# mihikamd/DP-GSAT

Hardware: AMD Instinct MI355X
Metric: million edges/s (attn+sample+aggregate fwd+bwd) (higher is better)
Workload: dtype f32

## Files before the change

### dp_gsat_amd/_lib.py

```python
from __future__ import annotations

import ctypes
import os
from ctypes import c_char_p, c_double, c_float, c_int, c_int32, c_int64, c_size_t, c_uint64, c_void_p

import torch

_HERE = os.path.dirname(os.path.abspath(__file__))
LIB_PATH = os.path.join(_HERE, "libgsat_hip.so")

P, I64, I32, F32, F64, SZ, INT, U64 = c_void_p, c_int64, c_int32, c_float, c_double, c_size_t, c_int, c_uint64

SIGNATURES = {
    "gsat_abi_version": (INT, []),
    "gsat_seed_next": (INT, [P, P, P]),
    "gsat_last_error": (c_char_p, []),
    "gsat_csr_workspace_bytes": (SZ, [I64, I64]),
    "gsat_rev_workspace_bytes": (SZ, [I64]),
    "gsat_build_csr": (INT, [P, P, I64, I64, P, P, P, P, P, SZ, P]),
    "gsat_reverse_edge_perm": (INT, [P, I64, I64, P, P, P, SZ, P]),
    "gsat_reverse_edge_perm_csr": (INT, [P, P, P, P, P, P, P, P, I64, I64, P, P, P]),
    "gsat_segment_ptr": (INT, [P, I64, I64, P, P, P]),
    "gsat_gather_i64": (INT, [P, I64, P, I64, P, P]),
    "gsat_row_chunks_workspace_bytes": (SZ, [I64]),
    "gsat_row_chunks": (INT, [P, I64, P, P, SZ, P]),
    "gsat_long_row_partial_floats": (SZ, [I64, I64]),
    "gsat_aggr_sum_fwd": (INT, [P, P, P, P, P, P, P, I64, I64, I64, F32, P, P, P, P]),
    "gsat_aggr_sum_bwd": (INT, [P, P, P, P, P, P, P, I64, I64, I64, F32, P, P, P, P, P, P]),
    "gsat_pna_fwd": (INT, [P, P, P, P, P, P, I64, I64, P, INT, P, INT, F32, F32, P, P]),
    "gsat_pna_bwd": (INT, [P, P, P, P, P, P, P, I64, I64, P, INT, P, INT, F32, F32, P, P, P, P, P]),
    "gsat_pna_long_row_floats": (SZ, [I64, I64, INT]),
    "gsat_pna_fwd_long": (INT, [P, P, P, P, P, P, I64, I64, I64, P, INT, P, INT, F32, F32, P, P, P, P]),
    "gsat_pna_bwd_long": (INT, [P, P, P, P, P, P, P, I64, I64, I64, P, INT, P, INT, F32, F32, P, P, P, P, P, P, P]),
    "gsat_pna_tile_plan": (INT, [I64, I64, P, P, P]),
    "gsat_pna_build_tiles": (INT, [P, P, P, P, P, I64, INT, INT, INT, P, P, P, P]),
    "gsat_pna_bwd_tiled": (INT, [P, P, P, P, P, P, P, I64, INT, INT, INT, P, P, I64, I64, I64, P, INT, P, INT, P, P, P, P, P, P, P]),
    "gsat_pna_fwd_compact": (INT, [P, P, P, P, P, I64, I64, P, INT, P, P, P]),
    "gsat_pna_post_fwd": (INT, [P, P, P, I64, I64, INT, P, I64, P, I64, P, P]),
    "gsat_pna_post_dw_workspace_floats": (SZ, [I64, I64, INT, I64]),
    "gsat_pna_post_dw": (INT, [P, P, P, I64, I64, INT, P, I64, P, P, SZ, P]),
    "gsat_pna_fwd_node_att": (INT, [P, P, P, P, I64, I64, P, INT, P, INT, F32, F32, P, P]),
    "gsat_pna_bwd_tiled_node_att": (INT, [P, P, P, P, P, P, I64, INT, INT, INT, P, P, I64, I64, I64, P, INT, P, INT, P, P, P, P, P, P, P, INT, P]),
    "gsat_csr_pair_workspace_bytes": (SZ, [I64, I64]),
    "gsat_build_csr_pair": (INT, [P, I64, I64] + [P] * 12 + [P, SZ, P]),
    "gsat_segment_ptr32": (INT, [P, I64, I64, P, P, P, P]),
    "gsat_bn_workspace_floats": (SZ, [I64, I64]),
    "gsat_bn_fwd": (INT, [P, P, P, P, P, I64, I64, INT, F32, F32, INT, P, P, P, P, P]),
    "gsat_bn_bwd": (INT, [P, P, P, P, P, P, I64, I64, INT, INT, P, P, P, P, P]),
    "gsat_bn_act_fwd": (INT, [P, P, P, P, P, I64, I64, INT, F32, F32, INT, P, F32, U64, P, P, P, P, P, P]),
    "gsat_bn_act_bwd": (INT, [P, P, P, P, P, P, I64, I64, INT, INT, F32, U64, P, P, P, P, P, P, P]),
    "gsat_bn_act_fwd_valid": (INT, [P, P, P, P, P, I64, I64, INT, F32, F32, INT, P, F32, U64, P, P, P, P, P, P, P]),
    "gsat_bn_act_bwd_valid": (INT, [P, P, P, P, P, P, I64, I64, INT, INT, F32, U64, P, P, P, P, P, P, P, P]),
    "gsat_bn_local_sum": (INT, [P, P, I64, I64, P, P, P]),
    "gsat_bn_apply_fwd": (INT, [P, P, P, P, P, I64, I64, INT, P, F32, U64, P, P, P]),
    "gsat_bn_local_bwd_sums": (INT, [P, P, P, P, P, P, I64, I64, INT, F32, U64, P, P, P, P, P]),
    "gsat_bn_apply_bwd": (INT, [P, P, P, P, P, P, P, P, I64, P, I64, I64, INT, F32, U64, P, P, P, P]),
    "gsat_relu_dropout_fwd": (INT, [P, I64, I64, F32, U64, P, P, P]),
    "gsat_relu_dropout_bwd": (INT, [P, P, I64, I64, F32, P, P]),
    "gsat_colsum_workspace_floats": (SZ, [I64]),
    "gsat_colsum": (INT, [P, I64, I64, P, P, P]),
    "gsat_embsum_fwd": (INT, [P, P, INT, P, I64, I64, P, P]),
    "gsat_onehot_rows": (INT, [P, P, INT, I64, I64, P, P]),
    "gsat_gemm_workspace_floats": (SZ, [INT, I64, I64, I64]),
    "gsat_gemm_plan": (INT, [INT, INT, INT, I64, I64, I64, INT, INT, I64, P]),
    "gsat_gemm_f32": (INT, [INT, INT, I64, I64, I64, P, I64, P, I64, P, I64, P, INT, P, SZ, P]),
    "gsat_gemm_bf16x3": (INT, [INT, INT, I64, I64, I64, P, I64, P, I64, P, I64, P, INT, P, SZ, P]),
    "gsat_attn_fwd_workspace_bytes": (SZ, [P]),
    "gsat_attn_fwd_kind": (I32, [P]),
    "gsat_attn_bwd_workspace_bytes": (SZ, [P]),
    "gsat_attn_fwd": (INT, [P, P]),
    "gsat_attn_bwd": (INT, [P, P, P]),
    "gsat_instance_norm_fwd": (INT, [P, P, P, P, I64, I64, I64, P, P, P]),
    "gsat_instance_norm_bwd": (INT, [P, P, P, P, P, P, I64, I64, I64, P, P, P]),
    "gsat_philox_keep_mask": (INT, [U64, I32, I64, I64, F32, P, P]),
    "gsat_philox_noise": (INT, [U64, I64, P, P]),
    "gsat_sample_fwd": (INT, [P, P, INT, F32, F32, I64, P, P]),
    "gsat_sample_bwd": (INT, [P, P, F32, I64, P, P]),
    "gsat_gumbel_sigmoid_philox": (INT, [P, I64, F32, F32, U64, P, P, P]),
    "gsat_philox_gumbel_noise": (INT, [U64, I64, P, P]),
    "gsat_lift_fwd": (INT, [P, P, P, I64, P, P]),
    "gsat_lift_bwd": (INT, [P, P, P, P, P, P, P, P, I64, P, P]),
    "gsat_symmetrise": (INT, [P, P, P, I64, P, P]),
    "gsat_info_loss_fwd": (INT, [P, P, F32, I64, P, P, P]),
    "gsat_info_loss_bwd": (INT, [P, P, F32, P, I64, P, P]),
    "gsat_info_loss_valid_fwd": (INT, [P, P, F32, P, I64, P, P, P, P]),
    "gsat_info_loss_valid_bwd": (INT, [P, P, F32, P, P, I64, P, P, P]),
    "gsat_f1_sparsity_fwd": (INT, [P, P, I64, P, P, P, P, P]),
    "gsat_f1_sparsity_bwd": (INT, [P, P, P, P, I64, P, P, P]),
    "gsat_f1_sparsity_block_entries": (I64, []),
    "gsat_f1_sparsity_max_blocks": (I64, []),
    "gsat_criterion_fwd": (INT, [P, P, I64, I64, INT, P, P, P, P, P]),
    "gsat_criterion_bwd": (INT, [P, P, P, P, I64, I64, INT, P, P, P]),
    "gsat_criterion_block_items": (I64, [I64, INT]),
    "gsat_criterion_max_blocks": (I64, []),
    "gsat_ragged_scan": (INT, [P, I64, P, P, I64, P, P, P, P, P, P]),
    "gsat_collate_padded_ragged": (INT, [P, I64, P, P, P, P, I64, P, P, I64, I64, P, P, P, P, P, P]),
    "gsat_collate_padded": (INT, [P, I64, P, P, P, I64, P, P, I64, I64, P, P, P, P, P, P]),
    "gsat_collate": (INT, [P, I64, P, P, P, I64, P, P, I64, I64, P, P, P, P, P]),
    "gsat_line_graph_pair_counts": (INT, [P, I64, P, P]),
    "gsat_line_graph": (INT, [P, P, P, I64, I64, P, P]),
    "gsat_narrow_i64": (INT, [P, I64, P, P]),
    "gsat_und_edges_workspace_bytes": (SZ, [I64]),
    "gsat_und_edges": (INT, [P, I64, I64, P, P, P, P, P, P, P, P, SZ, P]),
    "gsat_und_line_graph_counts": (INT, [P, P, P, P, I64, P, P]),
    "gsat_und_line_graph": (INT, [P, P, P, P, P, I64, I64, P, P]),
    "gsat_segment_pool_fwd": (INT, [P, P, I64, I64, INT, P, P]),
    "gsat_segment_pool_bwd": (INT, [P, P, I64, I64, INT, P, P]),
    "gsat_rank_edges_lds_cap": (I64, []),
    "gsat_rank_edges_workspace_bytes": (SZ, [I64]),
    "gsat_rank_edges": (INT, [P, P, P, P, I64, I64, I64, I64, INT, P, P, P, P, P, SZ, P]),
    "gsat_auroc_workspace_bytes": (SZ, [I64]),
    "gsat_auroc": (INT, [P, P, I64, P, P, SZ, P]),
    "gsat_delta_kl_workspace_bytes": (SZ, [I64]),
    "gsat_delta_kl": (INT, [P, P, I64, F64, P, P, SZ, P]),
    "gsat_auroc_tasks_workspace_bytes": (SZ, [I64, I64]),
    "gsat_auroc_tasks": (INT, [P, P, I64, I64, P, P, SZ, P]),
    "gsat_att_histogram": (INT, [P, P, I64, I64, F64, F64, P, P, P]),
    "gsat_subgraph_block_items": (I64, []),
    "gsat_subgraph_workspace_bytes": (SZ, [I64, I64]),
# ... 79 lines not shown
```

### dp_gsat_amd/csrc/attn.hip

```cpp
#include "common.h"
#include "attn_fused.h"
#include <cstdlib>

namespace gsat {

constexpr float IN_EPS = 1e-5f;
constexpr int SB = 256;
#ifndef GSAT_SB_LANES
#define GSAT_SB_LANES 16
#endif
constexpr int SB_LANES = GSAT_SB_LANES;
constexpr int SB_SLOTS = SB / SB_LANES;
constexpr int SB_RC = 2;

struct GemmWs { float* ptr; size_t floats; };
static int gemm_rm(hipStream_t stream, bool ta, bool tb, int64_t M, int64_t N, int64_t K, const float* A, int64_t lda, const float* B,
                   int64_t ldb, float beta, float* C, int64_t ldc, GemmWs ws = {nullptr, 0}, bool split_ok = false, SlabJob* defer = nullptr) {
    const char* env = getenv("GSAT_ATTN_BWD_SPLIT");
    const bool bwd_split = !(env && atoi(env) == 0);
    return gemm_f32(stream, ta, tb, M, N, K, A, lda, B, ldb, C, ldc, nullptr, beta != 0.f, ws.ptr, ws.floats, split_ok && bwd_split, defer);
}

template <bool EDGE>
struct PreAct {
    const float* P; const float* Q; const float* bias; const int32_t* src; const int32_t* dst; int C;
    __device__ __forceinline__ float4 load(int row, int c) const {
        float4 b = bias ? ld4(bias + c) : f4zero();
        float4 v;
        if (EDGE) {
            float4 p = ld4(P + (size_t)src[row] * C + c);
            float4 q = ld4(Q + (size_t)dst[row] * C + c);
            v = make_float4(p.x + q.x, p.y + q.y, p.z + q.z, p.w + q.w);
        } else {
            v = ld4(P + (size_t)row * C + c);
        }
        return make_float4(v.x + b.x, v.y + b.y, v.z + b.z, v.w + b.w);
    }
};

__device__ __forceinline__ float4 keep4(const float* mask, SeedRef sref, int layer, int row, int c, int C, float p, bool training) {
    if (!training || p <= 0.f) return make_float4(1.f, 1.f, 1.f, 1.f);
    if (mask) return ld4(mask + (size_t)row * C + c);
    return philox_keep4(sref.get(), layer, row, c, p);
}

__device__ __forceinline__ float4 slot_reduce(float4 v, float4 (*sm)[SB_LANES], int slot, int lane) {
    __syncthreads();
    sm[slot][lane] = v;
    __syncthreads();
    float4 r = f4zero();
    if (slot == 0) {
#pragma unroll
        for (int s = 0; s < SB_SLOTS; ++s) {
            float4 t = sm[s][lane];
            r.x += t.x; r.y += t.y; r.z += t.z; r.w += t.w;
        }
    }
    return r;
}

__device__ __forceinline__ void seg_slice(const int32_t* __restrict__ seg_ptr, int g, int* beg, int* end, float* inv_n) {
    const int b = seg_ptr[g], e = seg_ptr[g + 1];
    *inv_n = 1.f / (float)max(e - b, 1);
    const int Z = gridDim.z, z = blockIdx.z;
    if (Z > 1) {
        const int per = (e - b + Z - 1) / Z;
        *beg = min(e, b + z * per);
        *end = min(e, *beg + per);
    } else {
        *beg = b; *end = e;
    }
}
// ... 542 lines not shown
        const int m = (int)(i / C4), c = (int)(i % C4) * 4;
        st4(keep + (size_t)m * C + c, keep4(nullptr, SeedRef{seed, nullptr}, layer, m, c, C, p, true));
    }
}

static inline int ew_blocks(int64_t work_items) {
    int64_t nb = ceil_div(work_items, 256);
    if (nb > 256 * 32) nb = 256 * 32;
    return (int)std::max<int64_t>(nb, 1);
}

static int colsum(hipStream_t stream, const float* x, int64_t R, int C, float* out, float* scratch ) {
    if (C <= 0) return GSAT_OK;
    const int ctiles = (int)ceil_div(C, 4 * SB_LANES);
    if (R <= 0) { GSAT_CHECK_HIP(gsat::zero_async(out, sizeof(float) * C, stream)); return GSAT_OK; }
    int64_t RB = std::min<int64_t>(256, ceil_div(R, 64));
    if (RB <= 1) {
        k_colsum<<<dim3(ctiles, 1), SB, 0, stream>>>(x, R, C, R, out);
    } else {
        int64_t rpb = ceil_div(R, RB);
        RB = ceil_div(R, rpb);
        k_colsum<<<dim3(ctiles, (unsigned)RB), SB, 0, stream>>>(x, R, C, rpb, scratch);
        k_colsum<<<dim3(ctiles, 1), SB, 0, stream>>>(scratch, RB, C, RB, out);
    }
    GSAT_LAUNCH_CHECK();
    return GSAT_OK;
}

static inline int seg_slices(int64_t rows, int64_t G) {
    const int64_t avg = rows / std::max<int64_t>(G, 1);
    return (int)std::max<int64_t>(1, std::min<int64_t>(64, ceil_div(avg, 4096)));
}

template <bool EDGE>
static int launch_seg_stats(hipStream_t stream, PreAct<EDGE> pre, const int32_t* seg_ptr, const int32_t* order, int64_t G, int Z,
                            float* mean, float* rstd, float* part) {
    if (G <= 0) return GSAT_OK;
    const int C = pre.C;
    const dim3 grid((unsigned)G, (unsigned)ceil_div(C, 4 * SB_LANES), (unsigned)Z);
    if (Z == 1) {
        k_seg_stats<EDGE, false><<<grid, SB, 0, stream>>>(pre, seg_ptr, order, mean, rstd);
    } else {
        GSAT_REQUIRE(part, GSAT_ERR_WORKSPACE, "segmented statistics need a workspace for sliced segments");
        const unsigned cb = (unsigned)ceil_div(G * C, 256);
        k_seg_partial<EDGE><<<grid, SB, 0, stream>>>(pre, seg_ptr, order, nullptr, part);
        k_zcombine<<<cb, 256, 0, stream>>>(part, seg_ptr, (int)G, Z, C, 1, mean);
        k_seg_partial<EDGE><<<grid, SB, 0, stream>>>(pre, seg_ptr, order, mean, part);
        k_zcombine<<<cb, 256, 0, stream>>>(part, seg_ptr, (int)G, Z, C, 2, rstd);
    }
    GSAT_LAUNCH_CHECK();
    return GSAT_OK;
}

static size_t attn_gemm_ws_w2(const gsat_attn_args* a) { return align_up(gemm_workspace_floats(a->C2, a->C1, a->M, true), 64); }
static size_t attn_gemm_ws_w1(const gsat_attn_args* a) { return align_up(gemm_workspace_floats(a->C1, a->H, a->N, true), 64); }
static size_t attn_gemm_ws_floats(const gsat_attn_args* a) { return attn_gemm_ws_w2(a) + (a->edge_mode ? 2 : 1) * attn_gemm_ws_w1(a); }

static int check_args(const gsat_attn_args* a, const char* who) {
    GSAT_REQUIRE(a, GSAT_ERR_ARG, "%s: null args", who);
    GSAT_REQUIRE(a->M >= 0 && a->N >= 0 && a->G >= 0 && a->M < (1ll << 31) && a->N < (1ll << 31), GSAT_ERR_ARG, "%s: bad extents", who);
    GSAT_REQUIRE(a->H > 0 && a->C1 > 0 && a->C2 > 0 && a->H % 4 == 0 && a->C1 % 4 == 0 && a->C2 % 4 == 0, GSAT_ERR_UNSUPPORTED,
                 "%s: H, C1, C2 must be positive multiples of 4 (got %d, %d, %d)", who, a->H, a->C1, a->C2);
    GSAT_REQUIRE(a->p_drop >= 0.f && a->p_drop < 1.f, GSAT_ERR_ARG, "%s: dropout p must be in [0,1)", who);
    if (a->M == 0) return GSAT_OK;
    GSAT_REQUIRE(a->emb && a->W1 && a->b1 && a->W2 && a->b2 && a->W3 && a->b3 && a->seg_ptr && a->row_seg, GSAT_ERR_ARG, "%s: null input", who);
    GSAT_REQUIRE(a->P && a->h2 && a->stats && a->logits, GSAT_ERR_ARG, "%s: null output/saved buffer", who);
    if (a->edge_mode) GSAT_REQUIRE(a->src && a->dst && a->Q, GSAT_ERR_ARG, "%s: edge mode needs src, dst, Q", who);
    else GSAT_REQUIRE(a->M == a->N, GSAT_ERR_ARG, "%s: node mode needs M == N", who);
    return GSAT_OK;
}

}

using namespace gsat;

extern "C" {

size_t gsat_colsum_workspace_floats(int64_t C) { return (size_t)256 * (size_t)(C > 0 ? C : 0); }

int gsat_colsum(const float* x, int64_t R, int64_t C, float* out, float* workspace, void* stream) {
    GSAT_REQUIRE(R >= 0 && C >= 0 && C < (1ll << 31), GSAT_ERR_ARG, "gsat_colsum: bad extents");
    if (C == 0) return GSAT_OK;
    GSAT_REQUIRE(out && (x || R == 0) && workspace, GSAT_ERR_ARG, "gsat_colsum: null pointer");
    return colsum((hipStream_t)stream, x, R, (int)C, out, workspace);
}


int gsat_attn_fwd(const gsat_attn_args* a, void* stream_) {
    hipStream_t stream = (hipStream_t)stream_;
    int rc = check_args(a, "gsat_attn_fwd");
    if (rc) return rc;
    if (a->M == 0) return GSAT_OK;
    {
        FusedGeom fg;
        if (attn_fused_eligible(a, &fg)) return attn_fused_fwd(stream, a, fg);
    }
    GSAT_REQUIRE(a->a1, GSAT_ERR_ARG, "gsat_attn_fwd: the staged pipeline needs the a1 buffer");
    const int64_t M = a->M, N = a->N, G = a->G;
    const int H = a->H, C1 = a->C1, C2 = a->C2;
    float* mean1 = a->stats;
    float* rstd1 = mean1 + (size_t)G * C1;
    float* mean2 = rstd1 + (size_t)G * C1;
    float* rstd2 = mean2 + (size_t)G * C2;
    if (a->edge_mode) {
        if ((rc = gemm_rm(stream, false, true, N, C1, H, a->emb, H, a->W1, 2 * H, 0.f, a->P, C1))) return rc;
        if ((rc = gemm_rm(stream, false, true, N, C1, H, a->emb, H, a->W1 + H, 2 * H, 0.f, a->Q, C1))) return rc;
    } else {
        if ((rc = gemm_rm(stream, false, true, N, C1, H, a->emb, H, a->W1, H, 0.f, a->P, C1))) return rc;
// ... 281 lines not shown
```

### dp_gsat_amd/csrc/common.h

```cpp
#pragma once
#include <cstring>
#include <cstdint>
#include <cstdio>
#include <cstdarg>
#include <hip/hip_runtime.h>

#include "../../include/gsat_hip.h"

namespace gsat {

void set_error(const char* fmt, ...);
const char* get_error();

#define GSAT_CHECK_HIP(expr)                                                                  \
    do {                                                                                      \
        hipError_t _e = (expr);                                                               \
        if (_e != hipSuccess) {                                                               \
            gsat::set_error("%s:%d: %s -> %s", __FILE__, __LINE__, #expr, hipGetErrorString(_e)); \
            return GSAT_ERR_HIP;                                                              \
        }                                                                                     \
    } while (0)

#define GSAT_REQUIRE(cond, code, ...)                                                         \
    do {                                                                                      \
        if (!(cond)) {                                                                        \
            gsat::set_error(__VA_ARGS__);                                                     \
            return (code);                                                                    \
        }                                                                                     \
    } while (0)

#define GSAT_LAUNCH_CHECK() GSAT_CHECK_HIP(hipGetLastError())

static inline int64_t ceil_div(int64_t a, int64_t b) { return (a + b - 1) / b; }

hipError_t zero_async(void* p, size_t bytes, hipStream_t stream);
static inline size_t align_up(size_t a, size_t b) { return (a + b - 1) / b * b; }

struct Arena {
    char* base;
    size_t cap, off;
    Arena(void* p, size_t bytes) : base(static_cast<char*>(p)), cap(bytes), off(0) {}
    template <class T> T* take(size_t n) {
        size_t b = align_up(n * sizeof(T), 256);
        if (base == nullptr || off + b > cap) { off += b; return nullptr; }
        T* r = reinterpret_cast<T*>(base + off);
        off += b;
        return r;
    }
    bool ok() const { return base != nullptr && off <= cap; }
};

struct SlabJob { const float* ws; int nslab; size_t slab; int M, N; int64_t ldc; int accumulate; float* out; };
int gemm_f32(hipStream_t stream, bool a_t, bool b_t, int64_t M, int64_t N, int64_t K, const float* A, int64_t lda, const float* B,
             int64_t ldb, float* C, int64_t ldc, const float* bias, bool accumulate, float* ws, size_t ws_floats, bool allow_split = false,
             SlabJob* defer = nullptr);
int slab_reduce_jobs(hipStream_t stream, const SlabJob* jobs, int n);
size_t gemm_workspace_floats(int64_t M, int64_t N, int64_t K, bool reduce_rows);

int aggr_sum_fwd_impl(hipStream_t stream, const float* x, const float* self_rows, const float* att, const float* edge_emb,
                      const int32_t* rowptr, const int32_t* col, const int32_t* eid, int64_t N, int64_t E, int64_t H, float self_coef,
                      float* out, const int32_t* chunk_ptr, float* partial);

#ifdef __HIPCC__
constexpr int WAVE = 64;

template <int CTRL> __device__ __forceinline__ float dpp_add(float v) {
    const int t = __builtin_amdgcn_update_dpp(0, __builtin_bit_cast(int, v), CTRL, 0xF, 0xF, true);
    return v + __builtin_bit_cast(float, t);
}

template <int WIDTH> __device__ __forceinline__ float group_sum(float v) {
    if constexpr ((WIDTH & (WIDTH - 1)) == 0) {
        if constexpr (WIDTH >= 2) v = dpp_add<0xB1>(v);
        if constexpr (WIDTH >= 4) v = dpp_add<0x4E>(v);
        if constexpr (WIDTH >= 8) v = dpp_add<0x141>(v);
        if constexpr (WIDTH >= 16) v = dpp_add<0x140>(v);
        if constexpr (WIDTH >= 32) v += __builtin_bit_cast(float, __builtin_amdgcn_ds_swizzle(__builtin_bit_cast(int, v), 0x401F));
        if constexpr (WIDTH >= 64) v += __shfl_xor(v, 32, 64);
    } else {
        const int l = (int)(threadIdx.x & 63) % WIDTH;
#pragma unroll
        for (int o = 16; o > 0; o >>= 1) {
            const float t = __shfl_down(v, o, 64);
            if (l + o < WIDTH) v += t;
        }
    }
    return v;
}

template <int LPR, int BLOCK> struct LaneGroups {
    static constexpr int GPW = 64 / LPR, GPB = (BLOCK / 64) * GPW;
    int grp, lane;
    __device__ __forceinline__ LaneGroups() {
        const int wl = threadIdx.x & 63, sub = wl / LPR;
        lane = wl % LPR;
        grp = sub < GPW ? (int)(threadIdx.x >> 6) * GPW + sub : -1;
    }
};

__device__ __forceinline__ float4 ld4(const float* p) { return *reinterpret_cast<const float4*>(p); }
__device__ __forceinline__ void st4(float* p, float4 v) { *reinterpret_cast<float4*>(p) = v; }
__device__ __forceinline__ void st4_nt(float* p, float4 v) {
    typedef float v4f __attribute__((ext_vector_type(4)));
    v4f t = {v.x, v.y, v.z, v.w};
    __builtin_nontemporal_store(t, reinterpret_cast<v4f*>(p));
}
__device__ __forceinline__ float4 ld4_off(const float* base, uint32_t byte_off) {
    return *reinterpret_cast<const float4*>(reinterpret_cast<const char*>(base) + byte_off);
}
__device__ __forceinline__ void st4_off(float* base, uint32_t byte_off, float4 v) {
// ... 55 lines not shown
```

### dp_gsat_amd/csrc/gemm.hip

```cpp
#include "common.h"
#include "pna_math.h"
#include <cstdlib>

namespace gsat {

typedef float f32x16 __attribute__((ext_vector_type(16)));

constexpr int GK = 32, GT = 256;
constexpr int LD_KC = 129;
constexpr int LD_KM = 132;

struct StageKC { float4 v[4]; };
template <int ROWS>
__device__ __forceinline__ void load_kcontig(StageKC& s, const float* __restrict__ X, int64_t ld, int r0, int R, int k0, int K, int t) {
    const int kq = (t & 7) * 4;
#pragma unroll
    for (int p = 0; p < ROWS / 32; ++p) {
        const int r = r0 + (t >> 3) + 32 * p;
        s.v[p] = (r < R && k0 + kq < K) ? ld4(X + (size_t)r * ld + k0 + kq) : f4zero();
    }
}
template <int ROWS>
__device__ __forceinline__ void store_kcontig(const StageKC& s, float* __restrict__ L, int t) {
    const int kq = (t & 7) * 4;
// ... 874 lines not shown
    do {                                                                                                                            \
        if (split) {                                                                                                                \
            if (tm == 2 && tn == 2) k_gemm_bf16x3<AT, BT, 2, 2><<<grid, GT, 0, stream>>>(A, lda, B, ldb, out, ldo, (int)M, (int)N, (int)K, kps, bptr, acc_flag, slab); \
            else if (tm == 2) k_gemm_bf16x3<AT, BT, 2, 1><<<grid, GT, 0, stream>>>(A, lda, B, ldb, out, ldo, (int)M, (int)N, (int)K, kps, bptr, acc_flag, slab);       \
            else if (tn == 2) k_gemm_bf16x3<AT, BT, 1, 2><<<grid, GT, 0, stream>>>(A, lda, B, ldb, out, ldo, (int)M, (int)N, (int)K, kps, bptr, acc_flag, slab);       \
            else k_gemm_bf16x3<AT, BT, 1, 1><<<grid, GT, 0, stream>>>(A, lda, B, ldb, out, ldo, (int)M, (int)N, (int)K, kps, bptr, acc_flag, slab);                    \
        } else if (tm == 2 && tn == 2) k_gemm_f32<AT, BT, 2, 2><<<grid, GT, 0, stream>>>(A, lda, B, ldb, out, ldo, (int)M, (int)N, (int)K, kps, bptr, acc_flag, slab); \
        else if (tm == 2) k_gemm_f32<AT, BT, 2, 1><<<grid, GT, 0, stream>>>(A, lda, B, ldb, out, ldo, (int)M, (int)N, (int)K, kps, bptr, acc_flag, slab);       \
        else if (tn == 2) k_gemm_f32<AT, BT, 1, 2><<<grid, GT, 0, stream>>>(A, lda, B, ldb, out, ldo, (int)M, (int)N, (int)K, kps, bptr, acc_flag, slab);       \
        else k_gemm_f32<AT, BT, 1, 1><<<grid, GT, 0, stream>>>(A, lda, B, ldb, out, ldo, (int)M, (int)N, (int)K, kps, bptr, acc_flag, slab);                    \
    } while (0)
    if (a_t) { if (b_t) LAUNCH(true, true); else LAUNCH(true, false); }
    else { if (b_t) LAUNCH(false, true); else LAUNCH(false, false); }
#undef LAUNCH
    GSAT_LAUNCH_CHECK();
    if (splits > 1) {
        const bool vec = plan.reduce != 1 && ldc % 4 == 0 && slab % 4 == 0 && ((uintptr_t)C & 15) == 0 && ((uintptr_t)ws & 15) == 0;
        const int reduce = vec ? plan.reduce : 1;
        if (defer && vec) { *defer = SlabJob{ws, splits, slab, (int)M, (int)N, ldc, accumulate ? 1 : 0, C}; return GSAT_OK; }
        if (reduce == 16)
            k_slab_reduce4<16><<<(unsigned)ceil_div(M * N * 4, 256), 256, 0, stream>>>(ws, splits, slab, (int)M, (int)N, ldc, accumulate ? 1 : 0, C);
        else if (reduce == 8)
            k_slab_reduce4<8><<<(unsigned)ceil_div(M * N * 2, 256), 256, 0, stream>>>(ws, splits, slab, (int)M, (int)N, ldc, accumulate ? 1 : 0, C);
        else if (reduce == 4)
            k_slab_reduce4<4><<<(unsigned)ceil_div(M * N, 256), 256, 0, stream>>>(ws, splits, slab, (int)M, (int)N, ldc, accumulate ? 1 : 0, C);
        else
            k_slab_reduce<<<(unsigned)ceil_div(M * N, 256), 256, 0, stream>>>(ws, splits, slab, (int)M, (int)N, ldc, accumulate ? 1 : 0, C);
        GSAT_LAUNCH_CHECK();
    }
    return GSAT_OK;
}

int slab_reduce_jobs(hipStream_t stream, const SlabJob* jobs, int n) {
    SlabJobs4 J{};
    int m = 0, blocks = 0, wide = 0;
    for (int i = 0; i < n; ++i) wide = std::max(wide, jobs[i].nslab >= 128 ? 4 : (jobs[i].nslab >= 64 ? 2 : 0));
    for (int i = 0; i < n; ++i) {
        if (jobs[i].nslab <= 0) continue;
        GSAT_REQUIRE(m < 4, GSAT_ERR_ARG, "slab_reduce_jobs: more than four pending sums");
        J.job[m] = jobs[i];
        J.first[m] = blocks;
        blocks += (int)ceil_div((int64_t)jobs[i].M * jobs[i].N * (wide ? wide : 1), 256);
        ++m;
    }
    for (int q = m; q <= 4; ++q) J.first[q] = blocks;
    if (!blocks) return GSAT_OK;
    if (wide == 4) k_slab_reduce_jobs<16><<<blocks, 256, 0, stream>>>(J);
    else if (wide == 2) k_slab_reduce_jobs<8><<<blocks, 256, 0, stream>>>(J);
    else k_slab_reduce_jobs<4><<<blocks, 256, 0, stream>>>(J);
    GSAT_LAUNCH_CHECK();
    return GSAT_OK;
}

int pna_post_fwd(hipStream_t stream, const PnaVirt& pv, int64_t Nrows, const float* W, int64_t ldw, const float* bias, int64_t Ho, float* out, int64_t ldo) {
    const int64_t K = (int64_t)pv.NAGG * 2 * pv.H;
    GSAT_REQUIRE(pv.H % 32 == 0 && Ho % 4 == 0 && ldw % 4 == 0 && ldo % 4 == 0 && Nrows < (1ll << 31), GSAT_ERR_UNSUPPORTED, "gsat_pna_post_fwd: H must be a multiple of 32, Ho of 4");
    GSAT_REQUIRE(((uintptr_t)W % 16 == 0) && ((uintptr_t)out % 16 == 0) && (!bias || (uintptr_t)bias % 16 == 0) && ((uintptr_t)pv.x % 16 == 0) && ((uintptr_t)pv.aggj % 16 == 0),
                 GSAT_ERR_ARG, "gsat_pna_post_fwd: operands must be 16-byte aligned");
    if (Nrows <= 0 || Ho <= 0) return GSAT_OK;
    xcd_switch_once();
    const int tn = Ho > 64 ? 2 : 1;
    dim3 grid((unsigned)ceil_div(Ho, 64 * tn), (unsigned)ceil_div(Nrows, 128), 1);
    if (tn == 2) k_gemm_bf16x3<false, true, 2, 2, 1><<<grid, GT, 0, stream>>>(nullptr, 0, W, ldw, out, ldo, (int)Nrows, (int)Ho, (int)K, (int)K, bias, 0, 0, pv);
    else k_gemm_bf16x3<false, true, 2, 1, 1><<<grid, GT, 0, stream>>>(nullptr, 0, W, ldw, out, ldo, (int)Nrows, (int)Ho, (int)K, (int)K, bias, 0, 0, pv);
    GSAT_LAUNCH_CHECK();
    return GSAT_OK;
}

int pna_post_dw(hipStream_t stream, const PnaVirt& pv, int64_t Nrows, const float* dout, int64_t ldd, int64_t Ho, float* dW, int64_t lddw, float* ws,
                size_t ws_floats) {
    const int64_t Kc = (int64_t)pv.NAGG * 2 * pv.H;
    GSAT_REQUIRE(pv.H % 64 == 0 && Ho % 4 == 0 && ldd % 4 == 0 && lddw % 4 == 0 && Nrows < (1ll << 31), GSAT_ERR_UNSUPPORTED, "gsat_pna_post_dw: H must be a multiple of 64, Ho of 4");
    GSAT_REQUIRE(((uintptr_t)dout % 16 == 0) && ((uintptr_t)dW % 16 == 0) && ((uintptr_t)pv.x % 16 == 0) && ((uintptr_t)pv.aggj % 16 == 0), GSAT_ERR_ARG,
                 "gsat_pna_post_dw: operands must be 16-byte aligned");
    if (Ho <= 0) return GSAT_OK;
    xcd_switch_once();
    const int splits = gemm_splits(Ho, Kc, Nrows, true);
    const int tm = Ho <= 64 ? 1 : 2, tn = pv.H % 128 == 0 ? 2 : 1;
    dim3 grid((unsigned)ceil_div(Kc, 64 * tn), (unsigned)ceil_div(Ho, 64 * tm), (unsigned)splits);
    const int kps = (int)(ceil_div(ceil_div(Nrows, splits), GK) * GK);
    float* o = dW;
    int64_t ldo = lddw;
    size_t slab = 0;
    if (splits > 1) {
        GSAT_REQUIRE(ws && ws_floats >= (size_t)splits * Ho * Kc, GSAT_ERR_WORKSPACE, "gsat_pna_post_dw: split-K workspace too small");
        o = ws; ldo = Kc; slab = (size_t)Ho * Kc;
    }
#define GO(TM_, TN_) k_gemm_bf16x3<true, false, TM_, TN_, 2><<<grid, GT, 0, stream>>>(dout, ldd, nullptr, 0, o, ldo, (int)Ho, (int)Kc, (int)Nrows, kps, nullptr, 0, slab, pv)
    if (tm == 2 && tn == 2) GO(2, 2); else if (tm == 2) GO(2, 1); else if (tn == 2) GO(1, 2); else GO(1, 1);
#undef GO
    GSAT_LAUNCH_CHECK();
    if (splits > 1) {
        k_slab_reduce4<4><<<(unsigned)ceil_div(Ho * Kc, 256), 256, 0, stream>>>(ws, splits, slab, (int)Ho, (int)Kc, lddw, 0, dW);
        GSAT_LAUNCH_CHECK();
    }
    return GSAT_OK;
}

}

using namespace gsat;

extern "C" {

static int pna_virt_make(const char* who, const float* x, const float* aggj, const float* scal, int64_t H, int nagg, PnaVirt* pv) {
    GSAT_REQUIRE(x && aggj && scal && (nagg == 4 || nagg == 5) && H > 0 && ((uintptr_t)scal % 16 == 0), GSAT_ERR_ARG, "%s: bad aggregate operand", who);
    pv->x = x; pv->aggj = aggj; pv->scal = scal; pv->H = (int)H; pv->NAGG = nagg;
    return GSAT_OK;
}

int gsat_pna_post_fwd(const float* x, const float* aggj, const float* scal, int64_t N, int64_t H, int num_aggregators,
                      const float* W, int64_t ldw, const float* bias, int64_t Ho, float* out, void* stream) {
    PnaVirt pv;
    int rc = pna_virt_make("gsat_pna_post_fwd", x, aggj, scal, H, num_aggregators, &pv);
    if (rc) return rc;
    GSAT_REQUIRE(W && out, GSAT_ERR_ARG, "gsat_pna_post_fwd: null pointer");
    return pna_post_fwd((hipStream_t)stream, pv, N, W, ldw, bias, Ho, out, Ho);
}

size_t gsat_pna_post_dw_workspace_floats(int64_t N, int64_t H, int num_aggregators, int64_t Ho) {
    return gemm_workspace_floats(Ho, (int64_t)num_aggregators * 2 * H, N, true);
}

int gsat_pna_post_dw(const float* x, const float* aggj, const float* scal, int64_t N, int64_t H, int num_aggregators,
                     const float* dout, int64_t Ho, float* dW, float* workspace, size_t workspace_floats, void* stream) {
    PnaVirt pv;
    int rc = pna_virt_make("gsat_pna_post_dw", x, aggj, scal, H, num_aggregators, &pv);
    if (rc) return rc;
    GSAT_REQUIRE(dout && dW, GSAT_ERR_ARG, "gsat_pna_post_dw: null pointer");
    return pna_post_dw((hipStream_t)stream, pv, N, dout, Ho, Ho, dW, (int64_t)num_aggregators * 2 * H, workspace, workspace_floats);
}

int gsat_gemm_f32(int a_t, int b_t, int64_t M, int64_t N, int64_t K, const float* A, int64_t lda, const float* B, int64_t ldb,
                  float* C, int64_t ldc, const float* bias, int accumulate, float* workspace, size_t workspace_floats, void* stream) {
    return gemm_f32((hipStream_t)stream, a_t != 0, b_t != 0, M, N, K, A, lda, B, ldb, C, ldc, bias, accumulate != 0, workspace, workspace_floats, false);
}

int gsat_gemm_bf16x3(int a_t, int b_t, int64_t M, int64_t N, int64_t K, const float* A, int64_t lda, const float* B, int64_t ldb,
                     float* C, int64_t ldc, const float* bias, int accumulate, float* workspace, size_t workspace_floats, void* stream) {
    return gemm_f32((hipStream_t)stream, a_t != 0, b_t != 0, M, N, K, A, lda, B, ldb, C, ldc, bias, accumulate != 0, workspace, workspace_floats, true);
}

size_t gsat_gemm_workspace_floats(int a_t, int64_t M, int64_t N, int64_t K) { return gemm_workspace_floats(M, N, K, a_t != 0); }

int gsat_gemm_plan(int allow_split, int a_t, int b_t, int64_t M, int64_t N, int64_t K, int has_bias, int accumulate, int64_t ldb, int32_t* plan) {
    GSAT_REQUIRE(plan && M > 0 && N > 0 && K > 0, GSAT_ERR_ARG, "gsat_gemm_plan: bad argument");
    GSAT_REQUIRE(ldb % 4 == 0 && (a_t ? M % 4 == 0 : K % 4 == 0) && (b_t ? K % 4 == 0 : N % 4 == 0), GSAT_ERR_UNSUPPORTED,
                 "gsat_gemm_plan: contiguous extents and leading dimensions must be multiples of 4 (M=%lld N=%lld K=%lld)", (long long)M, (long long)N, (long long)K);
    const GemmPlan p = gemm_plan(allow_split != 0, a_t != 0, b_t != 0, M, N, K, has_bias != 0, accumulate != 0, ldb);
    GSAT_REQUIRE(!(has_bias && p.splits > 1), GSAT_ERR_UNSUPPORTED, "gsat_gemm_plan: bias with split-K");
    const int32_t v[8] = {p.family, p.tm, p.tn, p.splits, p.reduce, p.nb, p.kr, p.nq};
    memcpy(plan, v, sizeof(v));
    return GSAT_OK;
}

}
```

### include/gsat_hip.h

```cpp
#ifndef GSAT_HIP_H
#define GSAT_HIP_H

#include <stddef.h>
#include <stdint.h>

#ifdef __cplusplus
extern "C" {
#endif

#define GSAT_ABI_VERSION 4

#define GSAT_OK 0
#define GSAT_ERR_HIP (-1)
#define GSAT_ERR_ARG (-2)
#define GSAT_ERR_WORKSPACE (-3)
#define GSAT_ERR_UNSUPPORTED (-4)
#define GSAT_ERR_BLAS (-5)

int gsat_abi_version(void);

int gsat_seed_next(uint64_t* state, uint64_t* out, void* stream);
const char* gsat_last_error(void);


// ... 115 lines not shown
                int64_t N, int64_t C, int training, float momentum, float eps, int relu, float* y,
                float* save_mean, float* save_rstd, float* workspace, void* stream);
int gsat_bn_bwd(const float* x, const float* dy, const float* gamma, const float* beta, const float* save_mean,
                const float* save_rstd, int64_t N, int64_t C, int training, int relu, float* dx, float* dgamma,
                float* dbeta, float* workspace, void* stream);

int gsat_bn_act_fwd(const float* x, const float* gamma, const float* beta, float* running_mean, float* running_var,
                    int64_t N, int64_t C, int training, float momentum, float eps, int relu, const float* residual,
                    float dropout_p, uint64_t seed, const uint64_t* seed_dev, float* y, float* save_mean,
                    float* save_rstd, float* workspace, void* stream);
int gsat_bn_act_bwd(const float* x, const float* dy, const float* gamma, const float* beta, const float* save_mean,
                    const float* save_rstd, int64_t N, int64_t C, int training, int relu, float dropout_p,
                    uint64_t seed, const uint64_t* seed_dev, float* dx, float* dresidual, float* dgamma,
                    float* dbeta, float* workspace, void* stream);

int gsat_bn_act_fwd_valid(const float* x, const float* gamma, const float* beta, float* running_mean, float* running_var,
                          int64_t N, int64_t C, int training, float momentum, float eps, int relu, const float* residual,
                          float dropout_p, uint64_t seed, const uint64_t* seed_dev, float* y, float* save_mean,
                          float* save_rstd, float* workspace, const int32_t* n_valid_dev, void* stream);
int gsat_bn_act_bwd_valid(const float* x, const float* dy, const float* gamma, const float* beta, const float* save_mean,
                          const float* save_rstd, int64_t N, int64_t C, int training, int relu, float dropout_p,
                          uint64_t seed, const uint64_t* seed_dev, float* dx, float* dresidual, float* dgamma,
                          float* dbeta, float* workspace, const int32_t* n_valid_dev, void* stream);

int gsat_bn_local_sum(const float* x, const float* centre, int64_t N, int64_t C, float* out, float* workspace, void* stream);
int gsat_bn_apply_fwd(const float* x, const float* gamma, const float* beta, const float* mean, const float* rstd, int64_t N, int64_t C,
                      int relu, const float* residual, float dropout_p, uint64_t seed, const uint64_t* seed_dev, float* y, void* stream);
int gsat_bn_local_bwd_sums(const float* x, const float* dy, const float* gamma, const float* beta, const float* mean, const float* rstd,
                           int64_t N, int64_t C, int relu, float dropout_p, uint64_t seed, const uint64_t* seed_dev, float* sum_dy,
                           float* sum_dy_xhat, float* workspace, void* stream);
int gsat_bn_apply_bwd(const float* x, const float* dy, const float* gamma, const float* beta, const float* mean, const float* rstd,
                      const float* sum_dy, const float* sum_dy_xhat, int64_t global_rows, const float* global_rows_dev , int64_t N, int64_t C,
                      int relu, float dropout_p, uint64_t seed, const uint64_t* seed_dev, float* dx, float* dresidual, void* stream);

size_t gsat_colsum_workspace_floats(int64_t C);
int gsat_colsum(const float* x, int64_t R, int64_t C, float* out, float* workspace, void* stream);


int gsat_embsum_fwd(const int64_t* x, const int32_t* dims, int ncol, const float* W, int64_t N, int64_t H,
                    float* out, void* stream);
int gsat_onehot_rows(const int64_t* x, const int32_t* dims, int ncol, int64_t N, int64_t R_padded, float* O,
                     void* stream);


size_t gsat_gemm_workspace_floats(int a_t, int64_t M, int64_t N, int64_t K);
int gsat_gemm_plan(int allow_split, int a_t, int b_t, int64_t M, int64_t N, int64_t K, int has_bias, int accumulate,
                   int64_t ldb, int32_t* plan);
int gsat_gemm_f32(int a_t, int b_t, int64_t M, int64_t N, int64_t K, const float* A, int64_t lda,
                  const float* B, int64_t ldb, float* C, int64_t ldc, const float* bias, int accumulate,
                  float* workspace, size_t workspace_floats, void* stream);
int gsat_gemm_bf16x3(int a_t, int b_t, int64_t M, int64_t N, int64_t K, const float* A, int64_t lda,
                     const float* B, int64_t ldb, float* C, int64_t ldc, const float* bias, int accumulate,
                     float* workspace, size_t workspace_floats, void* stream);


typedef struct gsat_attn_args {
    int64_t M, N, G;
    int32_t H, C1, C2;
    int32_t edge_mode;
    int32_t training;
    float p_drop;
    uint64_t seed;
    const int32_t* src;
    const int32_t* dst;
    const int32_t* seg_ptr;
    const int32_t* seg_order;
    const int32_t* row_seg;
    const float *W1, *b1, *W2, *b2, *W3, *b3;
    const float* emb;
    const float* mask1;
    const float* mask2;
    const float* u;
    float* P;
    float* Q;
    float* a1;
    float* h2;
    float* stats;
    float* logits;
    float* att;
    void* fwd_workspace;
    size_t fwd_workspace_bytes;
    const uint64_t* seed_dev;
    int32_t noise_philox;
    int32_t fused;
    const int32_t* node_ptr;
} gsat_attn_args;

typedef struct gsat_attn_grads {
    const float* dlogits;
    const float* datt;
    const int32_t* rowptr_src;
    const int32_t* eid_by_src;
    const int32_t* rowptr_dst;
    const int32_t* eid_by_dst;
    const int32_t* chunk_ptr_src;
    const int32_t* chunk_ptr_dst;
    float *demb, *dW1, *db1, *dW2, *db2, *dW3, *db3;
    void* workspace;
    size_t workspace_bytes;
} gsat_attn_grads;

size_t gsat_attn_fwd_workspace_bytes(const gsat_attn_args* args);
int gsat_attn_fwd_kind(const gsat_attn_args* args);
size_t gsat_attn_bwd_workspace_bytes(const gsat_attn_args* args);
int gsat_attn_fwd(const gsat_attn_args* args, void* stream);
int gsat_attn_bwd(const gsat_attn_args* args, const gsat_attn_grads* grads, void* stream);
// ... 152 lines not shown
```

Baseline: 127.1.

## Add dedicated split-K bf16x3 MFMA kernel for attention weight-gradient GEMMs

Adds a specialised weight-gradient GEMM kernel (A^T·B with a long K) that uses 128x128 tiles, 512 threads, a three-register-stage prefetch with double-buffered LDS, and bf16x3 MFMA emulation of f32. The split count is chosen from the CU count so the grid fills the device, and partial tiles go to a workspace that the existing slab-reduce step sums. The attention backward routes eligible transposed-A GEMMs through it and sizes its workspace for it. Ineligible shapes fall back to the old path, and the extra splits can enlarge the workspace and the reduction traffic.

```diff
diff --git a/dp_gsat_amd/_lib.py b/dp_gsat_amd/_lib.py
--- a/dp_gsat_amd/_lib.py
+++ b/dp_gsat_amd/_lib.py
@@ -65,6 +65,8 @@
     "gsat_gemm_plan": (INT, [INT, INT, INT, I64, I64, I64, INT, INT, I64, P]),
     "gsat_gemm_f32": (INT, [INT, INT, I64, I64, I64, P, I64, P, I64, P, I64, P, INT, P, SZ, P]),
     "gsat_gemm_bf16x3": (INT, [INT, INT, I64, I64, I64, P, I64, P, I64, P, I64, P, INT, P, SZ, P]),
+    "gsat_gemm_wgrad_plan": (INT, [I64, I64, I64, P]),
+    "gsat_gemm_wgrad_x3": (INT, [I64, I64, I64, P, I64, P, I64, P, I64, INT, P, SZ, P]),
     "gsat_attn_fwd_workspace_bytes": (SZ, [P]),
     "gsat_attn_fwd_kind": (I32, [P]),
     "gsat_attn_bwd_workspace_bytes": (SZ, [P]),
diff --git a/dp_gsat_amd/csrc/attn.hip b/dp_gsat_amd/csrc/attn.hip
--- a/dp_gsat_amd/csrc/attn.hip
+++ b/dp_gsat_amd/csrc/attn.hip
@@ -18,6 +18,7 @@
                    int64_t ldb, float beta, float* C, int64_t ldc, GemmWs ws = {nullptr, 0}, bool split_ok = false, SlabJob* defer = nullptr) {
     const char* env = getenv("GSAT_ATTN_BWD_SPLIT");
     const bool bwd_split = !(env && atoi(env) == 0);
+    if (ta && !tb && split_ok && bwd_split) return gemm_wgrad(stream, M, N, K, A, lda, B, ldb, C, ldc, beta != 0.f, ws.ptr, ws.floats, defer);
     return gemm_f32(stream, ta, tb, M, N, K, A, lda, B, ldb, C, ldc, nullptr, beta != 0.f, ws.ptr, ws.floats, split_ok && bwd_split, defer);
 }
 
@@ -666,8 +667,8 @@
     return GSAT_OK;
 }
 
-static size_t attn_gemm_ws_w2(const gsat_attn_args* a) { return align_up(gemm_workspace_floats(a->C2, a->C1, a->M, true), 64); }
-static size_t attn_gemm_ws_w1(const gsat_attn_args* a) { return align_up(gemm_workspace_floats(a->C1, a->H, a->N, true), 64); }
+static size_t attn_gemm_ws_w2(const gsat_attn_args* a) { return align_up(gemm_wgrad_workspace_floats(a->C2, a->C1, a->M), 64); }
+static size_t attn_gemm_ws_w1(const gsat_attn_args* a) { return align_up(gemm_wgrad_workspace_floats(a->C1, a->H, a->N), 64); }
 static size_t attn_gemm_ws_floats(const gsat_attn_args* a) { return attn_gemm_ws_w2(a) + (a->edge_mode ? 2 : 1) * attn_gemm_ws_w1(a); }
 
 static int check_args(const gsat_attn_args* a, const char* who) {
diff --git a/dp_gsat_amd/csrc/common.h b/dp_gsat_amd/csrc/common.h
--- a/dp_gsat_amd/csrc/common.h
+++ b/dp_gsat_amd/csrc/common.h
@@ -56,6 +56,11 @@
              SlabJob* defer = nullptr);
 int slab_reduce_jobs(hipStream_t stream, const SlabJob* jobs, int n);
 size_t gemm_workspace_floats(int64_t M, int64_t N, int64_t K, bool reduce_rows);
+struct WgradPlan { int eligible, S, rows; size_t ws_floats; };
+WgradPlan wgrad_plan(int64_t Mo, int64_t No, int64_t K);
+size_t gemm_wgrad_workspace_floats(int64_t Mo, int64_t No, int64_t K);
+int gemm_wgrad(hipStream_t stream, int64_t Mo, int64_t No, int64_t K, const float* A, int64_t lda, const float* B, int64_t ldb, float* C,
+               int64_t ldc, bool accumulate, float* ws, size_t ws_floats, SlabJob* defer = nullptr);
 
 int aggr_sum_fwd_impl(hipStream_t stream, const float* x, const float* self_rows, const float* att, const float* edge_emb,
                       const int32_t* rowptr, const int32_t* col, const int32_t* eid, int64_t N, int64_t E, int64_t H, float self_coef,
diff --git a/dp_gsat_amd/csrc/gemm.hip b/dp_gsat_amd/csrc/gemm.hip
--- a/dp_gsat_amd/csrc/gemm.hip
+++ b/dp_gsat_amd/csrc/gemm.hip
@@ -950,6 +950,165 @@
     return GSAT_OK;
 }
 
+constexpr int WG_T = 512, WG_TILE = 128;
+constexpr int WG_PLANE = (GK / 8) * WG_TILE * 16;
+constexpr int WG_BUF = 4 * WG_PLANE;
+constexpr int WG_MIN_SLABS = 8;
+
+__global__ __launch_bounds__(WG_T) void k_wgrad_x3(const float* A, int64_t lda, const float* B, int64_t ldb, float* ws, int Mo, int No, int K,
+                                                   int rows_per) {
+    constexpr int EP_LD = 36;
+    static_assert(2 * WG_BUF >= 8 * 32 * EP_LD * 4, "epilogue staging must fit in the operand planes");
+    __shared__ __attribute__((aligned(16))) unsigned char lds[2 * WG_BUF];
+    const int t = threadIdx.x, lane = t & 63, wave = t >> 6;
+    int bx, by, bz;
+    gemm_tile_coords(bx, by, bz);
+    const int m0 = by * WG_TILE, n0 = bx * WG_TILE;
+    const int kbeg = bz * rows_per, kend = min(K, kbeg + rows_per);
+    const int nslab = (kend - kbeg + GK - 1) / GK;
+    const int ts = t & 255, cp = (ts & 63) * 2, k8 = ts >> 6;
+    const bool stage_b = t >= 256;
+    const float* const src = stage_b ? B + n0 + cp : A + m0 + cp;
+    const int64_t ld = stage_b ? ldb : lda;
+    const int plane0 = stage_b ? 2 * WG_PLANE : 0;
+    auto gload = [&](StageKM& s, int slab) {
+        const int kb = kbeg + slab * GK + k8 * 8;
+#pragma unroll
+        for (int j = 0; j < 8; ++j) s.v[j] = *reinterpret_cast<const float2*>(src + (size_t)min(kb + j, kend - 1) * ld);
+    };
+    auto lstore = [&](StageKM& s, int slab, unsigned char* buf) {
+        const int kb = kbeg + slab * GK + k8 * 8;
+#pragma unroll
+        for (int j = 0; j < 8; ++j) s.v[j] = kb + j < kend ? s.v[j] : make_float2(0.f, 0.f);
+        store_split_kmajor<WG_TILE>(s, buf + plane0, buf + plane0 + WG_PLANE, ts);
+    };
+    f32x16 acc[2];
+#pragma unroll
+    for (int j = 0; j < 2; ++j)
+#pragma unroll
+        for (int r = 0; r < 16; ++r) acc[j][r] = 0.f;
+    const int r32 = lane & 31, kh = lane >> 5, wm = wave >> 1, wn = wave & 1;
+    auto compute = [&](const unsigned char* buf) {
+#pragma unroll
+        for (int ks = 0; ks < 2; ++ks) {
+            const int ko = (2 * ks + kh) * WG_TILE;
+            const int ao = (ko + wm * 32 + r32) * 16;
+            const bf16x8 ah = *reinterpret_cast<const bf16x8*>(buf + ao);
+            const bf16x8 al = *reinterpret_cast<const bf16x8*>(buf + WG_PLANE + ao);
+            bf16x8 bh[2], bl[2];
+#pragma unroll
+            for (int j = 0; j < 2; ++j) {
+                const int bo = (ko + wn * 64 + 32 * j + r32) * 16;
+                bh[j] = *reinterpret_cast<const bf16x8*>(buf + 2 * WG_PLANE + bo);
+                bl[j] = *reinterpret_cast<const bf16x8*>(buf + 3 * WG_PLANE + bo);
+            }
+#pragma unroll
+            for (int j = 0; j < 2; ++j) {
+                acc[j] = __builtin_amdgcn_mfma_f32_32x32x16_bf16(al, bl[j], acc[j], 0, 0, 0);
+                acc[j] = __builtin_amdgcn_mfma_f32_32x32x16_bf16(al, bh[j], acc[j], 0, 0, 0);
+                acc[j] = __builtin_amdgcn_mfma_f32_32x32x16_bf16(ah, bl[j], acc[j], 0, 0, 0);
+                acc[j] = __builtin_amdgcn_mfma_f32_32x32x16_bf16(ah, bh[j], acc[j], 0, 0, 0);
+            }
+        }
+    };
+    StageKM s0, s1, s2;
+    gload(s0, 0); gload(s1, 1); gload(s2, 2);
+    lstore(s0, 0, lds);
+    gload(s0, 3);
+    __syncthreads();
+    unsigned char* cur = lds;
+    unsigned char* nxt = lds + WG_BUF;
+    auto step = [&](int i, StageKM& s) {
+        compute(cur);
+        lstore(s, i + 1, nxt);
+        gload(s, i + 4);
+        __syncthreads();
+        unsigned char* tmp = cur; cur = nxt; nxt = tmp;
+    };
+    int i = 0;
+    for (; i + 3 <= nslab; i += 3) {
+        step(i, s1);
+        step(i + 1, s2);
+        step(i + 2, s0);
+    }
+    if (i < nslab) {
+        compute(cur);
+        if (i + 1 < nslab) {
+            lstore(s1, i + 1, nxt);
+            __syncthreads();
+            compute(nxt);
+        }
+        __syncthreads();
+    }
+    float* const Cb = ws + (size_t)bz * Mo * No;
+    float* const patch = reinterpret_cast<float*>(lds) + wave * (32 * EP_LD);
+    const int prow = lane >> 3, pcol = (lane & 7) * 4;
+#pragma unroll
+    for (int j = 0; j < 2; ++j) {
+#pragma unroll
+        for (int r = 0; r < 16; ++r) patch[((r & 3) + 8 * (r >> 2) + 4 * kh) * EP_LD + r32] = acc[j][r];
+        __builtin_amdgcn_wave_barrier();
+        const int col = n0 + wn * 64 + j * 32 + pcol;
+#pragma unroll
+        for (int p = 0; p < 4; ++p) {
+            const int rr = prow + 8 * p;
+            st4(Cb + (size_t)(m0 + wm * 32 + rr) * No + col, ld4(patch + rr * EP_LD + pcol));
+        }
+        __builtin_amdgcn_wave_barrier();
+    }
+}
+
+static int device_cus() {
+    static const int n = [] {
+        int dev = 0, v = 0;
+        if (hipGetDevice(&dev) != hipSuccess || hipDeviceGetAttribute(&v, hipDeviceAttributeMultiprocessorCount, dev) != hipSuccess || v <= 0) {
+            (void)hipGetLastError();
+            v = 256;
+        }
+        return v;
+    }();
+    return n;
+}
+
+WgradPlan wgrad_plan(int64_t Mo, int64_t No, int64_t K) {
+    WgradPlan p{};
+    if (Mo <= 0 || No <= 0 || K <= 0) return p;
+    p.S = gemm_splits(Mo, No, K, true);
+    p.rows = (int)std::min<int64_t>(ceil_div(ceil_div(K, p.S), GK) * GK, INT32_MAX);
+    p.ws_floats = gemm_workspace_floats(Mo, No, K, true);
+    if (Mo % WG_TILE != 0 || No % WG_TILE != 0 || K >= (1ll << 31) - 8 * GK || !use_bf16x3(Mo, No, K, true)) return p;
+    const int64_t tiles = (Mo / WG_TILE) * (No / WG_TILE), s0 = device_cus() / tiles;
+    if (s0 < 2 || K < s0 * WG_MIN_SLABS * GK) return p;
+    const int64_t rows = ceil_div(ceil_div(K, s0), GK) * GK;
+    p.eligible = 1;
+    p.rows = (int)rows;
+    p.S = (int)ceil_div(K, rows);
+    p.ws_floats = (size_t)p.S * Mo * No;
+    return p;
+}
+
+size_t gemm_wgrad_workspace_floats(int64_t Mo, int64_t No, int64_t K) {
+    return std::max(wgrad_plan(Mo, No, K).ws_floats, gemm_workspace_floats(Mo, No, K, true));
+}
+
+int gemm_wgrad(hipStream_t stream, int64_t Mo, int64_t No, int64_t K, const float* A, int64_t lda, const float* B, int64_t ldb, float* C,
+               int64_t ldc, bool accumulate, float* ws, size_t ws_floats, SlabJob* defer) {
+    const WgradPlan p = wgrad_plan(Mo, No, K);
+    if (!p.eligible) return gemm_f32(stream, true, false, Mo, No, K, A, lda, B, ldb, C, ldc, nullptr, accumulate, ws, ws_floats, true, defer);
+    if (defer) defer->nslab = 0;
+    xcd_switch_once();
+    GSAT_REQUIRE(A && B && C && lda >= Mo && ldb >= No && ldc >= No && lda % 4 == 0 && ldb % 4 == 0 && ldc % 4 == 0, GSAT_ERR_ARG, "gemm_wgrad: bad argument");
+    GSAT_REQUIRE(((uintptr_t)A % 16 == 0) && ((uintptr_t)B % 16 == 0) && ((uintptr_t)C % 16 == 0) && ((uintptr_t)ws % 16 == 0), GSAT_ERR_ARG,
+                 "gemm_wgrad: operands, output and workspace must be 16-byte aligned");
+    GSAT_REQUIRE(ws && ws_floats >= p.ws_floats, GSAT_ERR_WORKSPACE, "gemm_wgrad: workspace too small");
+    const dim3 grid((unsigned)(No / WG_TILE), (unsigned)(Mo / WG_TILE), (unsigned)p.S);
+    k_wgrad_x3<<<grid, WG_T, 0, stream>>>(A, lda, B, ldb, ws, (int)Mo, (int)No, (int)K, p.rows);
+    GSAT_LAUNCH_CHECK();
+    const SlabJob job{ws, p.S, (size_t)Mo * No, (int)Mo, (int)No, ldc, accumulate ? 1 : 0, C};
+    if (defer) { *defer = job; return GSAT_OK; }
+    return slab_reduce_jobs(stream, &job, 1);
+}
+
 int pna_post_fwd(hipStream_t stream, const PnaVirt& pv, int64_t Nrows, const float* W, int64_t ldw, const float* bias, int64_t Ho, float* out, int64_t ldo) {
     const int64_t K = (int64_t)pv.NAGG * 2 * pv.H;
     GSAT_REQUIRE(pv.H % 32 == 0 && Ho % 4 == 0 && ldw % 4 == 0 && ldo % 4 == 0 && Nrows < (1ll << 31), GSAT_ERR_UNSUPPORTED, "gsat_pna_post_fwd: H must be a multiple of 32, Ho of 4");
@@ -1041,6 +1200,20 @@
 
 size_t gsat_gemm_workspace_floats(int a_t, int64_t M, int64_t N, int64_t K) { return gemm_workspace_floats(M, N, K, a_t != 0); }
 
+int gsat_gemm_wgrad_plan(int64_t Mo, int64_t No, int64_t K, int32_t* plan) {
+    GSAT_REQUIRE(plan && Mo > 0 && No > 0 && K > 0, GSAT_ERR_ARG, "gsat_gemm_wgrad_plan: bad argument");
+    const WgradPlan p = wgrad_plan(Mo, No, K);
+    GSAT_REQUIRE(p.ws_floats <= (size_t)INT32_MAX, GSAT_ERR_UNSUPPORTED, "gsat_gemm_wgrad_plan: workspace of %zu floats does not fit int32", p.ws_floats);
+    const int32_t v[4] = {p.eligible, p.S, p.rows, (int32_t)p.ws_floats};
+    memcpy(plan, v, sizeof(v));
+    return GSAT_OK;
+}
+
+int gsat_gemm_wgrad_x3(int64_t Mo, int64_t No, int64_t K, const float* A, int64_t lda, const float* B, int64_t ldb, float* C, int64_t ldc,
+                       int accumulate, float* workspace, size_t workspace_floats, void* stream) {
+    return gemm_wgrad((hipStream_t)stream, Mo, No, K, A, lda, B, ldb, C, ldc, accumulate != 0, workspace, workspace_floats);
+}
+
 int gsat_gemm_plan(int allow_split, int a_t, int b_t, int64_t M, int64_t N, int64_t K, int has_bias, int accumulate, int64_t ldb, int32_t* plan) {
     GSAT_REQUIRE(plan && M > 0 && N > 0 && K > 0, GSAT_ERR_ARG, "gsat_gemm_plan: bad argument");
     GSAT_REQUIRE(ldb % 4 == 0 && (a_t ? M % 4 == 0 : K % 4 == 0) && (b_t ? K % 4 == 0 : N % 4 == 0), GSAT_ERR_UNSUPPORTED,
diff --git a/include/gsat_hip.h b/include/gsat_hip.h
--- a/include/gsat_hip.h
+++ b/include/gsat_hip.h
@@ -191,6 +191,9 @@
 int gsat_gemm_bf16x3(int a_t, int b_t, int64_t M, int64_t N, int64_t K, const float* A, int64_t lda,
                      const float* B, int64_t ldb, float* C, int64_t ldc, const float* bias, int accumulate,
                      float* workspace, size_t workspace_floats, void* stream);
+int gsat_gemm_wgrad_plan(int64_t Mo, int64_t No, int64_t K, int32_t* plan);
+int gsat_gemm_wgrad_x3(int64_t Mo, int64_t No, int64_t K, const float* A, int64_t lda, const float* B, int64_t ldb,
+                       float* C, int64_t ldc, int accumulate, float* workspace, size_t workspace_floats, void* stream);
 
 
 typedef struct gsat_attn_args {
```

Result: faster. 129.3, median of 6 (+1.8%).
